# wcy199705/DfFintheWild

Measured on AMD Instinct MI355X. Metric: focal-stacks/sec (10x3x256x256), higher is better.
Workload: dtype bf16x3 (split-bf16 MFMA operands hi+lo, fp32 accumulate, fp32-accurate); 1 GPU; DFF_net forward, 10-slice 3x256x256 focal stacks, batch 32 per GPU (BASELINE.json config 3), dense focus_dists, synthetic weights seed 0; batch_per_gpu=32, global_batch=32, slices=10, height=256, width=256, parallelism=single GPU, precision=bf16x3, input=float32 (B,3,N,H,W), the reference's tensor contract

## Files before the change

dffinthewild_amd/csrc/dffw_dispatch.cpp:

```cpp
#include "dffw_run.h"
#include "dffw_stem.h"

namespace dffw {
namespace {

struct ConvLaunch {
    char kernel[96];
    const char *suffix;
    ConvArgs a;
    RollArgs r;
    int v0, v1;
    double flops, bytes;
};

enum { F_TILE = 100, F_GATHER = 101 };

struct ConvPlan {
    int family = -1;
    int n = 0;
    ConvLaunch l[4];
    bool clear_scores = false;
    const TileCfg *cfg = nullptr;
    TileArgs t;
    bool stem_pipe = false;
// ... 441 lines not shown
    }
    const PackedConv &pc = it->second;
    const LayerDef &L = pc.def;
    const int cin = in0.C + (o.in1 ? o.in1->C : 0);
    if (cin != pc.cin_all) {
        err = fail(DFFW_EINVAL, "layer %s expects %d input channels, got %d", name.c_str(), pc.cin_all, cin);
        return out;
    }
    int Ho, Wo;
    if (L.transposed) {
        Ho = in0.H * 2;
        Wo = in0.W * 2;
    } else {
        const int win = (L.kh == 9 && L.cin == 3) ? in0.W - 2 : in0.W;
        Ho = (in0.H + 2 * L.ph - L.dh * (L.kh - 1) - 1) / L.sh + 1;
        Wo = (win + 2 * L.pw - L.dw * (L.kw - 1) - 1) / L.sw + 1;
    }
    const int No = in0.N + 2 * L.pd - (L.kd - 1);
    if (o.outf == nullptr && !o.discard && !o.sums) out = act(in0.B, No, Ho, Wo, L.cout);
    else { out.B = in0.B; out.N = No; out.H = Ho; out.W = Wo; out.C = L.cout; }
    if (o.out_pre) *o.out_pre = act(in0.B, No, Ho, Wo, L.cout);
    if (!ok()) return out;

    const PackedConv *cls = nullptr;
    if (o.cls) {
        auto ic = e->convs.find(o.cls);
        if (ic != e->convs.end()) cls = &ic->second;
    }
    ConvPlan p;
    plan_conv(name, pc, cls, in0, o, out, sw, e->prec, p);
    if (p.err != DFFW_OK) {
        err = fail(p.err, "%s", p.msg);
        return out;
    }
    float *partial = p.partial_bytes ? (float *)raw(p.partial_bytes) : nullptr;
    if (!ok()) return out;
    if (dry) {
        drop_raw(partial);
        return out;
    }

    const uint16_t *zero = zero_page();
    if (!zero) return out;
    if (p.clear_scores) check(hipMemsetAsync(o.cls_out, 0, (size_t)out.pixels() * 4, s), "score memset");
    const StreamFamily *f = p.family < kStreamCount ? &kStream[p.family] : nullptr;
    const size_t trace_words = p.family == F_TILE ? (size_t)p.t.total_tiles * 8 : (f && f->step_trace) ? STEP_TRACE_WORDS : 0;
    p.t.partial = partial;
    for (int i = 0; i < p.n; ++i) {
        ConvLaunch &l = p.l[i];
        l.a.zero = zero;
        launch(l.kernel, name, l.suffix, l.flops, l.bytes, name.c_str(), trace_words, [&](unsigned long long *trace) {
            l.a.trace = trace;
            if (f) return f->go(e->prec, l, s);
            if (p.family == F_GATHER) return launch_conv(e->prec, l.a, s);
            return p.stem_pipe ? launch_stem_pipe(l.a, p.t, sw.roll_wgs, s) : launch_conv_tile(e->prec, p.cfg, l.a, p.t, s);
        });
    }
    if (partial) {
        launch_unnamed("dffw::splitk_finish_kernel", name, " (split-K finish)", 0.0, p.finish_bytes, "splitk_finish", 0, [&](unsigned long long *) {
#if defined(DFFW_ABL_BUILD) && defined(DFFW_EXP_SKIP_FINISH)
            return hipSuccess;
#endif
            return launch_splitk_finish(e->prec, partial, p.t.ksplit, p.t.partial_stride, p.M_out, pc.nt * 16, L.cout, pc.bias, p.l[0].a.res0, o.relu, out.p, s);
        });
        drop_raw(partial);
    }
    trace_end();
    return out;
}

}
```

dffinthewild_amd/csrc/dffw_engine.cpp:

```cpp
#include <algorithm>
#include <cmath>
#include <cstdarg>
#include <cstdio>
#include <cstdlib>
#include <cstring>
#include <map>
#include <memory>
#include <string>
#include <vector>

#include "dffw_run.h"
#include "dffw_srd_roll.h"
#include "dffw_stem.h"

namespace dffw {

static thread_local std::string g_err;
static thread_local std::string g_last_kernel;
static thread_local std::string g_last_op_kernels;
}
int dffw_fail(int code, const char *fmt, ...) {
    char buf[1024];
    va_list ap;
    va_start(ap, fmt);
// ... 201 lines not shown
                SrdArgs a = srd_args(x.p, out.p, c0->second, c2->second, x.B, x.N, x.H, x.W, sty, stx, r.sw.srd_wgs);
                if (!(a.zero = r.zero_page())) return out;
                a.pooled = with_pool ? pooled->p : nullptr;
                a.w3 = a3->second.w32; a.w1 = a1->second.w32;
                a.w3f = a3->second.watt; a.w1f = a1->second.watt;
                char kn[64];
                const bool pipe16 = x.C == 16 && r.sw.srd_pipe;
                if (pipe16) srd_pipe16_kernel_name(r.e->prec, with_pool, kn, sizeof kn);
                else if (x.C == 16) srd_roll16_kernel_name(r.e->prec, with_pool, kn, sizeof kn);
                else srd_roll_kernel_name(r.e->prec, with_pool, kn, sizeof kn);
                const double px = (double)x.pixels();
                r.launch(kn, p, "", 2.0 * px * (2 * 9 + 4) * x.C * x.C, (with_pool ? 2.25 : 2.0) * px * x.C * r.elem_bytes(), "srd_roll", SRD_TRACE_WORDS, [&](unsigned long long *trace) {
#ifdef DFFW_TRACE_BUILD
                    a.trace = trace;
#endif
                    return pipe16 ? launch_srd_pipe16(r.e->prec, a, r.s) : x.C == 16 ? launch_srd_roll16(r.e->prec, a, r.s) : launch_srd_roll(r.e->prec, a, r.s);
                });
                r.trace_end();
            }
            if (drop_x) r.drop(x);
            return out;
        }
    }
    ConvOpt o1; o1.relu = 1;
    Act t = r.conv(p + ".Focus_Measure.conv.0.0", x, o1);
    ConvOpt o2; o2.relu = 1; o2.res0 = &x;
    Act feat = r.conv(p + ".Focus_Measure.conv.2.0", t, o2);
    r.drop(t);
    if (drop_x) r.drop(x);
    Act out;
    auto i3 = r.e->convs.find(p + ".N_ch_attention.0");
    auto i1 = r.e->convs.find(p + ".N_ch_attention.2");
    if (srd_attention_supported(feat.C) && i3 != r.e->convs.end() && i1 != r.e->convs.end() && i3->second.w32 && i1->second.w32 &&
        !r.sw.on(SW_NO_FUSED_ATTENTION)) {
        out = r.act(feat.B, feat.N, feat.H, feat.W, feat.C);
        const bool with_pool = pooled && !r.sw.on(SW_NO_FUSED_POOL);
        if (with_pool) *pooled = r.act(feat.B, feat.N, feat.H / 2, feat.W / 2, feat.C);
        if (r.ok() && !r.dry) {
            char kn[64];
            snprintf(kn, sizeof kn, "dffw::srd_attention_kernel<%d, %d>", r.e->prec, feat.C);
            const double px = (double)feat.pixels();
            r.launch_unnamed(kn, p, ".N_ch_attention", 2.0 * px * 4 * feat.C * feat.C, (with_pool ? 2.25 : 2.0) * px * feat.C * r.elem_bytes(), "srd_attention", 0, [&](unsigned long long *) {
                return launch_srd_attention(r.e->prec, feat.p, out.p, i3->second.w32, i1->second.w32, feat.B, feat.N, feat.H, feat.W, feat.C, with_pool ? pooled->p : nullptr, r.s);
            });
        }
    } else if (feat.C == 32 && i3 != r.e->convs.end() && i1 != r.e->convs.end() && i3->second.watt && i1->second.watt && feat.W % 16 == 0 &&
               !r.sw.on(SW_NO_FUSED_ATTENTION)) {
        out = r.act(feat.B, feat.N, feat.H, feat.W, feat.C);
        if (r.ok() && !r.dry) {
            char kn[64];
            snprintf(kn, sizeof kn, "dffw::srd_attention_mfma<%d>", r.e->prec);
            const double px = (double)feat.pixels();
            r.launch_unnamed(kn, p, ".N_ch_attention", 2.0 * px * 4 * feat.C * feat.C, 2.0 * px * feat.C * r.elem_bytes(), "srd_attention_mfma", 0, [&](unsigned long long *) {
                return launch_srd_attention_mfma(r.e->prec, feat.p, out.p, i3->second.watt, i1->second.watt, feat.B, feat.N, feat.H, feat.W, r.s);
            });
        }
    } else {
        ConvOpt o3; o3.relu = 1;
        Act a = r.conv(p + ".N_ch_attention.0", feat, o3);
        ConvOpt o4; o4.relu = 2; o4.res0 = &feat;
        out = r.conv(p + ".N_ch_attention.2", a, o4);
        r.drop(a);
    }
    r.drop(feat);
    return out;
}

Act efd(Run &r, const std::string &p, const Act &x, Act *pooled) {
    auto ca = r.e->convs.find(p + ".stride_conv.0"), cb = r.e->convs.find(p + ".max_pooling.1.0");
    const int Ho = x.H / 2, Wo = x.W / 2;
    const double opx = (double)x.B * x.N * Ho * Wo;
    auto fused = [&](int C, int ty, int tx) {
        return x.C == C && pooled && pooled->p && ca != r.e->convs.end() && cb != r.e->convs.end() && x.H % 2 == 0 && x.W % 2 == 0 && Ho % ty == 0 && Wo % tx == 0 &&
               (int64_t)x.B * (Ho / ty) * (Wo / tx) >= r.sw.roll_min_units && !r.sw.on(SW_NO_ROLL) && !r.sw.on(SW_NO_FUSED_EFD) && !r.sw.on(SW_NO_TILE);
    };
    auto args = [&](int cout, uint16_t *out) {
        ConvArgs a;
        memset(&a, 0, sizeof a);
        a.in0 = x.p; a.C0 = x.C;
        a.in1 = pooled->p; a.C1 = x.C;
        a.B = x.B; a.Ni = x.N; a.Hi = x.H; a.Wi = x.W;
        a.Ng = x.N; a.Hg = Ho; a.Wg = Wo;
        a.No = x.N; a.Ho = Ho; a.Wo = Wo;
        a.Cout = cout;
        a.bias = ca->second.bias;
        a.out = out;
        a.relu = 1;
        a.M = (int64_t)x.B * x.N * Ho * Wo;
        return a;
    };
    int ty, tx;
    efd_roll_tile(&ty, &tx);
    if (fused(8, ty, tx) && ca->second.wroll8 && cb->second.wroll8) {
        Act out = r.act(x.B, x.N, Ho, Wo, 16);
        if (r.ok() && !r.dry) {
            ConvArgs a = args(16, out.p);
            if (!(a.zero = r.zero_page())) return out;
            a.dbg = (r.sw.debug_flags & 6) | r.sw.path_bits();
            RollArgs t = roll_args(ca->second.wroll8, x.B, Ho / ty, Wo / tx, 1, r.sw.roll_wgs);
            t.wroll2 = cb->second.wroll8;
            t.bias2 = cb->second.bias;
            char kn[64];
            conv_roll_efd_kernel_name(r.e->prec, a, true, kn, sizeof kn);
            r.launch(kn, p, "", 2.0 * opx * 27.0 * 8 * 16 * 2, ((double)x.pixels() * 8 + opx * 8 + opx * 16) * r.elem_bytes(), "conv_roll_efd", 0,
                     [&](unsigned long long *) { return launch_conv_roll_efd(r.e->prec, a, t, r.s); });
        }
        r.drop(*pooled);
// ... 520 lines not shown
```

dffinthewild_amd/csrc/dffw_internal.h:

```cpp
#pragma once
#include <hip/hip_runtime.h>
#include <stdint.h>

int dffw_fail(int code, const char *fmt, ...);
void dffw_set_last_op_kernels(const char *names);

namespace dffw {

struct Act {
    uint16_t *p = nullptr;
    int B = 0, N = 0, H = 0, W = 0, C = 0;
    int64_t pixels() const { return (int64_t)B * N * H * W; }
};

enum Prec { P_BF16X3 = 0, P_FP16 = 1, P_BF16 = 2 };
inline int prec_parts(int prec) { return prec == P_BF16X3 ? 2 : 1; }

struct TapEntry {
    int dz, dy, dx;
    int coff;
};
static_assert(sizeof(TapEntry) == 16, "TapEntry must be 16 bytes");

#define DFFW_TAP_INVALID (1 << 20)

struct RawStack {
    const void *p;
    int dtype;
    int64_t sb, sn, sy, sx, sc;
    int h, w;
};

#define DFFW_RAW_NORM_F64_BIT 16
#define DFFW_ARGS_RAW 8
#define DFFW_ARGS_SUMS 128
#define DFFW_ARGS_NO_SMALL 32
#define DFFW_ARGS_NO_LEAN_TILE 16
#define DFFW_ARGS_NO_LEAN_ROLL 64
#define DFFW_ARGS_NO_ROLLX 256
#define DFFW_ARGS_NO_SLICE32 1024
#define DFFW_ARGS_NO_ROLLT 2048
#define DFFW_ARGS_NO_ROLLK 512
struct ConvArgs {
    const uint16_t *in0, *in1;
    int C0, C1;
    int B, Ni, Hi, Wi;
    int Ng, Hg, Wg;
    int sy, sx;
    int No, Ho, Wo;
    int osy, osx, ooy, oox;
    int Cout, KC;
    const TapEntry *tab;
    const uint16_t *wpk;
    const float *bias;
    const uint16_t *res0, *res1;
    int res_bcast;
    uint16_t *out;
    uint16_t *out_pre;
    float *outf;
    int outf_ch;
    int64_t outf_plane;
    const float *cls_w;
    float *cls_out;
    int relu;
    int dbg;
    const uint16_t *zero;
    const float *fs32;
    unsigned long long *trace;
    int64_t M;
};

int conv_nt_for(int cout);
hipError_t launch_conv(int prec, const ConvArgs &a, hipStream_t s);
void conv_kernel_name_for(int prec, const ConvArgs &a, char *buf, int n);
hipError_t launch_set_raw(const RawStack &rs, RawStack *dst, hipStream_t s);
hipError_t launch_stack_in(int prec, const float *FS, uint16_t *out, int B, int N, int H, int W, hipStream_t s);
hipError_t launch_from_ncdhw(int prec, const float *x, uint16_t *out, int B, int C, int N, int H, int W, hipStream_t s);
hipError_t launch_to_ncdhw(int prec, const uint16_t *x, float *out, int B, int C, int N, int H, int W, hipStream_t s);
hipError_t launch_pool(int prec, int mode, int k, const uint16_t *x, uint16_t *out, int B, int N, int H, int W, int C, hipStream_t s);
hipError_t launch_pool3(int prec, const uint16_t *x, uint16_t *o2, uint16_t *o4, uint16_t *o8, int B, int N, int H, int W, int C, hipStream_t s);
bool srd_attention_supported(int C);
hipError_t launch_srd_attention(int prec, const uint16_t *feat, uint16_t *out, const float *w3, const float *w1, int B, int N,
                                int H, int W, int C, uint16_t *pooled, hipStream_t s);
hipError_t launch_splitk_finish(int prec, const float *partial, int ksplit, int64_t stride, int64_t M, int cpad, int Cout,
                                const float *bias, const uint16_t *res0, int relu, uint16_t *out, hipStream_t s);
hipError_t launch_from_ncdhw_pad(int prec, const float *x, uint16_t *out, int B, int Cs, int C, int N, int H, int W, hipStream_t s);
hipError_t launch_flow_volume(int prec, const uint16_t *fe, uint16_t *out, const float *alpha, const float *fov, int B, int N,
                              int H, int W, int C, int mode, hipStream_t s);
hipError_t launch_alpha_mean(const float *head, float *alpha, float *raw, int B, int N, int64_t hw, hipStream_t s);
int head_tail_chunks(int B, int N, int64_t hw);
hipError_t launch_head_tail_rows(const float *rows, double *seg, int tiles_x, const float *w, float *alpha, float *raw, int B, int N, int H, int W,
                                 int C, hipStream_t s);
int64_t head_tail_tiles_scratch_bytes(int B, int N, int C);
hipError_t launch_head_tail_tiles(const float *tsum, double *seg, int tiles_y, int tiles_x, const float *w, float *alpha, float *raw, int B,
                                  int N, int H, int W, int C, hipStream_t s);
hipError_t launch_head_tail(int prec, const uint16_t *v, double *partial, const float *w, float *alpha, float *raw, int B, int N, int H, int W,
                            int C, hipStream_t s);
hipError_t launch_fov_warp(const float *x, const float *alpha, const float *fov, float *out, float *flow, int B, int C, int N,
                           int H, int W, int alpha_from_sample0, hipStream_t s);
struct RegressHeads {
    const float *score[4];
    float *depth[4];
    int h[4], w[4];
    int n;
    int nofuse;
};
int regress_form(const RegressHeads &hd, int B, int N, int H, int W);
const char *regress_kernel_name(const RegressHeads &hd, int B, int N, int H, int W);
hipError_t launch_regress_heads(const RegressHeads &hd, int B, int N, int H, int W, const float *fd, int64_t fsb, int64_t fsn, int64_t fsh,
                                int64_t fsw, hipStream_t s);
hipError_t launch_regress(const float *score, int B, int N, int h, int w, int H, int W, const float *fd,
                          int64_t fsb, int64_t fsn, int64_t fsh, int64_t fsw, float *depth, hipStream_t s);

}
```

dffinthewild_amd/csrc/dffw_kernels.hip:

```cpp
#include <cstdio>
#include <cstdlib>

#include "dffw_device.h"
#include "dffw_internal.h"
#include "dffw_persist.h"

namespace dffw {

template <int PREC, int NT, int MT>
__global__ __launch_bounds__(256) void conv_igemm(const ConvArgs a) {
    constexpr int PARTS = Fmt<PREC>::PARTS;
    constexpr bool F16 = (PREC == P_FP16);
    const int lane = threadIdx.x & 63;
    const int wave = threadIdx.x >> 6;
    const int g = lane >> 4, r = lane & 15;
    const int64_t pos0 = ((int64_t)blockIdx.x * 4 + wave) * (MT * 16);
    if (pos0 >= a.M) return;

    const int ps0 = PARTS * a.C0, ps1 = PARTS * a.C1;
    const int64_t samp0 = (int64_t)a.Ni * a.Hi * a.Wi * ps0;
    const int64_t samp1 = (int64_t)a.Ni * a.Hi * a.Wi * ps1;

    int pn[MT], py[MT], px[MT], pbase[MT];
    bool pv[MT];
    int64_t opix[MT];
    const uint16_t *s0[MT];
    const uint16_t *s1[MT];
#pragma unroll
    for (int mt = 0; mt < MT; ++mt) {
        const int64_t p = pos0 + mt * 16 + r;
        pv[mt] = p < a.M;
        const int64_t pp = pv[mt] ? p : 0;
        const int x = (int)(pp % a.Wg);
        int64_t t = pp / a.Wg;
        const int y = (int)(t % a.Hg);
        t /= a.Hg;
        const int n = (int)(t % a.Ng);
        const int b = (int)(t / a.Ng);
        pn[mt] = n;
        py[mt] = y * a.sy;
        px[mt] = x * a.sx;
        pbase[mt] = (n * a.Hi + py[mt]) * a.Wi + px[mt];
        s0[mt] = a.in0 + b * samp0;
        s1[mt] = a.in1 + b * samp1;
        opix[mt] = (((int64_t)b * a.No + n) * a.Ho + (y * a.osy + a.ooy)) * a.Wo + (x * a.osx + a.oox);
    }

    f32x4 acc[NT][MT];
#pragma unroll
    for (int nt = 0; nt < NT; ++nt)
#pragma unroll
        for (int mt = 0; mt < MT; ++mt) acc[nt][mt] = f32x4{0.f, 0.f, 0.f, 0.f};

    const short8 *wbase = reinterpret_cast<const short8 *>(a.wpk) + lane;
    const short8 zero8 = short8{0, 0, 0, 0, 0, 0, 0, 0};

    for (int kc = 0; kc < a.KC; ++kc) {
        const TapEntry te = a.tab[kc * 4 + g];
        const bool tvalid = te.coff >= 0;
        const bool second = te.coff >= a.C0;
        const int cc = tvalid ? (second ? te.coff - a.C0 : te.coff) : 0;
        const int ps = second ? ps1 : ps0;
        const int csrc = second ? a.C1 : a.C0;
        const int delta = (te.dz * a.Hi + te.dy) * a.Wi + te.dx;

// ... 96 lines not shown
                f32x4 &pa = (i & 1) ? acc2 : acc, &qa = (i & 1) ? acc : acc2;
                if constexpr (PARTS == 2) {
                    pa = mma<F16>(wf[i][1], xh[i], pa);
                    qa = mma<F16>(wf[i][0], xl[i], qa);
                }
                pa = mma<F16>(wf[i][0], xh[i], pa);
            }
        }
    }
#pragma unroll
    for (int i = 0; i < 4; ++i) acc[i] += acc2[i];
    if constexpr (KS > 1) {
        red[wave][lane] = acc;
        __syncthreads();
        if (wave != 0) return;
#pragma unroll
        for (int w = 1; w < KS; ++w) {
            const f32x4 o = red[w][lane];
            acc[0] += o[0]; acc[1] += o[1]; acc[2] += o[2]; acc[3] += o[3];
        }
    }
    float cls = 0.f;
    epilogue_quad<PREC, false>(a, acc, nt, g, opix, pv, cls, uint4{}, uint4{});
}

static bool conv_small_wanted(const ConvArgs &a) {
    const int64_t tiles = (a.M + 15) / 16;
    return !a.cls_w && tiles <= 4096 && a.KC >= 1;
}

int conv_nt_for(int cout) {
    const int nt = (cout + 15) / 16;
    return nt <= 1 ? 1 : nt <= 2 ? 2 : nt <= 4 ? 4 : 8;
}

using ConvRow = KernelRow<ConvArgs>;
#define R(P) DFFW_ROW(64, conv_small, P, 1), DFFW_ROW(128, conv_small, P, 2), DFFW_ROW(256, conv_small, P, 4), DFFW_ROW(512, conv_small, P, 8)
static const ConvRow kSmall[] = {R(0), R(1), R(2)};
#undef R
struct IgemmRow {
    ConvRow row;
    int mt;
};
#define R_(P, NT, MT) {DFFW_ROW(256, conv_igemm, P, NT, MT), MT}
#define R(P) R_(P, 1, 4), R_(P, 2, 4), R_(P, 4, 4), R_(P, 8, 2)
static const IgemmRow kIgemm[] = {R(0), R(1), R(2)};
#undef R
#undef R_

struct ConvChoice {
    const ConvRow *row;
    dim3 grid;
};
static ConvChoice select_conv(int prec, const ConvArgs &a) {
    const int nt = conv_nt_for(a.Cout);
    if (conv_small_wanted(a) && !(a.dbg & DFFW_ARGS_NO_SMALL))
        return {prec_row(kSmall, prec, 4, a.KC >= 8 ? 3 : a.KC >= 4 ? 2 : a.KC >= 2 ? 1 : 0), dim3((unsigned)((a.M + 15) / 16), (unsigned)nt)};
    const IgemmRow *r = a.Cout <= 8 * 16 ? prec_row(kIgemm, prec, 4, nt == 8 ? 3 : nt == 4 ? 2 : nt == 2 ? 1 : 0) : nullptr;
    if (!r) return {nullptr, dim3()};
    const int64_t per_wg = 4 * r->mt * 16;
    return {&r->row, dim3((unsigned)((a.M + per_wg - 1) / per_wg))};
}

hipError_t launch_conv(int prec, const ConvArgs &a, hipStream_t s) {
    const ConvChoice c = select_conv(prec, a);
    if (!c.row) return hipErrorInvalidValue;
    hipLaunchKernelGGL(c.row->fn, c.grid, dim3(c.row->block), 0, s, a);
    return hipGetLastError();
}

void conv_kernel_name_for(int prec, const ConvArgs &a, char *buf, int n) { copy_row_name(select_conv(prec, a).row, buf, n); }

template <int PREC>
__global__ __launch_bounds__(256) void stack_in_kernel(const float *__restrict__ FS, uint16_t *__restrict__ out, int B,
                                                       int N, int H, int W) {
    constexpr int PARTS = Fmt<PREC>::PARTS;
    const int W2 = W + 2;
    const int64_t plane = (int64_t)N * H * W;
    const int64_t total = (int64_t)B * N * H * W2;
    for (int64_t i = (int64_t)blockIdx.x * blockDim.x + threadIdx.x; i < total; i += (int64_t)gridDim.x * blockDim.x) {
        const int q = (int)(i % W2);
        const int64_t row = i / W2;
        const int64_t b = row / ((int64_t)N * H);
        const int64_t nh = row - b * (int64_t)N * H;
        const float *src = FS + b * 3 * plane + nh * W;
        short8 h = short8{0, 0, 0, 0, 0, 0, 0, 0}, l = h;
#pragma unroll
        for (int c = 0; c < 3; ++c) {
            uint16_t hi, lo;
            Fmt<PREC>::split(q >= 2 ? src[c * plane + q - 2] : 0.f, hi, lo);
            h[c] = (short)hi;
            l[c] = (short)lo;
            Fmt<PREC>::split(q < W ? src[c * plane + q] : 0.f, hi, lo);
            h[4 + c] = (short)hi;
            l[4 + c] = (short)lo;
        }
        short8 *dst = reinterpret_cast<short8 *>(out + i * (PARTS * 8));
        dst[0] = h;
        if constexpr (PARTS == 2) dst[1] = l;
    }
}

template <int PREC>
__global__ __launch_bounds__(256) void from_ncdhw_kernel(const float *__restrict__ x, uint16_t *__restrict__ out, int B,
                                                         int C, int64_t plane) {
    constexpr int PARTS = Fmt<PREC>::PARTS;
    const int64_t total = (int64_t)B * plane * C;
    for (int64_t i = (int64_t)blockIdx.x * blockDim.x + threadIdx.x; i < total; i += (int64_t)gridDim.x * blockDim.x) {
        const int c = (int)(i % C);
        const int64_t pix = i / C;
        const int64_t b = pix / plane, q = pix - b * plane;
        Fmt<PREC>::store(out + pix * (PARTS * C), C, c, x[(b * C + c) * plane + q]);
    }
}

template <int PREC>
__global__ __launch_bounds__(256) void from_ncdhw_pad_kernel(const float *__restrict__ x, uint16_t *__restrict__ out, int B,
                                                             int Cs, int C, int64_t plane) {
    constexpr int PARTS = Fmt<PREC>::PARTS;
    if (C == 8) {
        const int64_t npix = (int64_t)B * plane;
        for (int64_t pix = (int64_t)blockIdx.x * blockDim.x + threadIdx.x; pix < npix; pix += (int64_t)gridDim.x * blockDim.x) {
            const int64_t b = pix / plane, q = pix - b * plane;
            short8 h = short8{0, 0, 0, 0, 0, 0, 0, 0}, l = h;
// ... 948 lines not shown
```

dffinthewild_amd/csrc/dffw_srd_roll.h:

```cpp
#pragma once
#include "dffw_internal.h"

namespace dffw {

struct SrdArgs {
    const uint16_t *x;
    uint16_t *out;
    uint16_t *pooled;
    const uint16_t *w0, *w2;
    const float *b0, *b2;
    const float *w3, *w1;
    const uint16_t *w3f, *w1f;
    const uint16_t *zero;
    int B, N, H, W;
    int tiles_y, tiles_x, total_tiles;
    int wgs;
#ifdef DFFW_TRACE_BUILD
    unsigned long long *trace;
#endif
};

constexpr int SRD_CHUNKS = 3;
void srd_roll_tile(int *ty, int *tx);
hipError_t launch_srd_roll(int prec, const SrdArgs &a, hipStream_t s);
void srd_roll_kernel_name(int prec, bool pool, char *buf, int n);
constexpr int SRD16_CHUNKS = 5;
void srd_roll16_tile(int *ty, int *tx);
hipError_t launch_srd_roll16(int prec, const SrdArgs &a, hipStream_t s);
void srd_roll16_kernel_name(int prec, bool pool, char *buf, int n);
hipError_t launch_srd_pipe16(int prec, const SrdArgs &a, hipStream_t s);
void srd_pipe16_kernel_name(int prec, bool pool, char *buf, int n);

hipError_t launch_srd_attention_mfma(int prec, const uint16_t *feat, uint16_t *out, const uint16_t *w3f, const uint16_t *w1f, int B, int N,
                                     int H, int W, hipStream_t s);

}
```

dffinthewild_amd/csrc/dffw_srd_roll.hip:

```cpp
#include <algorithm>
#include <cstdio>
#include <cstdlib>
#include <type_traits>

#include "dffw_device.h"
#include "dffw_persist.h"
#include "dffw_srd_roll.h"

namespace dffw {

using SrdRow = KernelRow<SrdArgs>;

template <int PREC, bool POOL, int ABL = 0>
__global__ __launch_bounds__(256) __attribute__((amdgpu_waves_per_eu(3))) void srd_roll_kernel(const SrdArgs a, const float *__restrict__ w3g, const float *__restrict__ w1g) {
    constexpr int PARTS = Fmt<PREC>::PARTS;
    constexpr bool F16 = (PREC == P_FP16);
    constexpr int C = 8, TY = 8, TX = 16, NWAVES = 4;
    constexpr int XY = TY + 4, XX = TX + 4, XPIX = XY * XX;
    constexpr int TYT = TY + 2, TXT = TX + 2, TPIX = TYT * TXT;
    constexpr int PIXB = C * 2;
    constexpr int NPIECE = (XPIX + 63) / 64;
    constexpr int PLANEB = NPIECE * 1024;
    constexpr int SLOTB = PARTS * PLANEB;
    constexpr int RX = 4;
// ... 1022 lines not shown
                Fmt<PREC>::join2(h23, l23, m[2], m[3]);
                uint32_t ph01, ph23, pl01, pl23;
#pragma unroll
                for (int i = 0; i < 4; ++i) {
                    uint32_t mu = __float_as_uint(m[i]);
                    mu = max(mu, (uint32_t)__builtin_amdgcn_mov_dpp((int)mu, 0xB1, 0xF, 0xF, true));
                    mu = max(mu, (uint32_t)__builtin_amdgcn_mov_dpp((int)mu, 0x128, 0xF, 0xF, true));
                    m[i] = __uint_as_float(mu);
                }
                Fmt<PREC>::split2(m[0], m[1], ph01, pl01);
                Fmt<PREC>::split2(m[2], m[3], ph23, pl23);
                if constexpr (PARTS == 2) {
                    swap16(ph01, pl01);
                    swap16(ph23, pl23);
                }
                if ((r & 9) == 0 && !(ABL & 32)) {
                    const int64_t pp = (((int64_t)UC.b * a.N + zC) * (a.H / 2) + (UC.gy0 / 2 + (wave >> 1))) * (a.W / 2) + UC.gx0 / 2 + 4 * (wave & 1) + ((r & 7) >> 1);
                    if constexpr (PARTS == 2) *reinterpret_cast<uint4 *>(a.pooled + pp * rec + (g & 1) * C + (g >> 1) * 8) = make_uint4(ph01, ph23, pl01, pl23);
                    else *reinterpret_cast<uint2 *>(a.pooled + pp * rec + g * 4) = make_uint2(ph01, ph23);
                }
            }
            if constexpr (PARTS == 2) {
                swap16(h01, l01);
                swap16(h23, l23);
                if ((ABL & 32) == 0 || h01 == 0x12345u) *reinterpret_cast<uint4 *>(a.out + pix * rec + (g & 1) * C + (g >> 1) * 8) = make_uint4(h01, h23, l01, l23);
            } else {
                *reinterpret_cast<uint2 *>(a.out + pix * rec + g * 4) = make_uint2(h01, h23);
            }
        }
        UC = UB;
        zC = zB;
        UB = UA;
        zB = zA;
        if (hasA) {
            xslot = (xslot + 1 == RX) ? 0 : xslot + 1;
            if (++zA == a.N) {
                zA = 0;
                cuA += wgs_per_xcd;
                if (cuA < uend) UA = decode(cuA);
            }
        }
    }
    asm volatile("s_waitcnt vmcnt(0)" ::: "memory");
}

template <int PREC>
__global__ __launch_bounds__(256) void srd_attention_mfma(const uint16_t *__restrict__ feat, uint16_t *__restrict__ out,
                                                          const uint16_t *__restrict__ w3f, const uint16_t *__restrict__ w1f, int B, int N,
                                                          int H, int W) {
    constexpr int PARTS = Fmt<PREC>::PARTS;
    constexpr bool F16 = (PREC == P_FP16);
    constexpr int C = 32, REC = PARTS * C;
    const int lane = threadIdx.x & 63, g = lane >> 4, r = lane & 15;
    const int64_t strip = (int64_t)blockIdx.x * 4 + (threadIdx.x >> 6);
    const int strips_per_row = W / 16;
    const int64_t nstrips = (int64_t)B * H * strips_per_row;
    if (strip >= nstrips) return;
    const int sx = (int)(strip % strips_per_row);
    const int64_t by = strip / strips_per_row;
    const int y = (int)(by % H), b = (int)(by / H);
    const int64_t hw = (int64_t)H * W;
    const int64_t pix0 = ((int64_t)b * N * H + y) * W + sx * 16 + r;

    short8 w3[3][2][PARTS], w1[2][2][2];
#pragma unroll
    for (int k = 0; k < 3; ++k)
#pragma unroll
        for (int nt = 0; nt < 2; ++nt)
#pragma unroll
            for (int pt = 0; pt < PARTS; ++pt) w3[k][nt][pt] = reinterpret_cast<const short8 *>(w3f)[((k * 2 + nt) * PARTS + pt) * 64 + lane];
#pragma unroll
    for (int c = 0; c < 2; ++c)
#pragma unroll
        for (int fr = 0; fr < PARTS; ++fr)
#pragma unroll
            for (int nt = 0; nt < 2; ++nt) w1[c][fr][nt] = reinterpret_cast<const short8 *>(w1f)[((c * PARTS + fr) * 2 + nt) * 64 + lane];

    auto load = [&](int z, short8 (&f)[PARTS]) {
#pragma unroll
        for (int pt = 0; pt < PARTS; ++pt) f[pt] = short8{0, 0, 0, 0, 0, 0, 0, 0};
        if ((unsigned)z < (unsigned)N) {
            const uint16_t *p = feat + (pix0 + (int64_t)z * hw) * REC + g * 8;
#pragma unroll
            for (int pt = 0; pt < PARTS; ++pt) f[pt] = *reinterpret_cast<const short8 *>(p + pt * C);
        }
    };
    auto load_res = [&](int z, uint2 (&rh)[2], uint2 (&rl)[2]) {
#pragma unroll
        for (int nt = 0; nt < 2; ++nt) {
            rh[nt] = make_uint2(0, 0);
            rl[nt] = make_uint2(0, 0);
            if (z < N) {
                const uint16_t *cp = feat + (pix0 + (int64_t)z * hw) * REC + nt * 16 + g * 4;
                rh[nt] = *reinterpret_cast<const uint2 *>(cp);
                if constexpr (PARTS == 2) rl[nt] = *reinterpret_cast<const uint2 *>(cp + C);
            }
        }
    };
    short8 f[4][PARTS];
    uint2 rh[2][2], rl[2][2];
    load(-1, f[0]);
    load(0, f[1]);
    load(1, f[2]);
    load_res(0, rh[0], rl[0]);
    for (int z = 0; z < N; ++z) {
        load(z + 2, f[3]);
        load_res(z + 1, rh[1], rl[1]);
        f32x4 at[2];
#pragma unroll
        for (int nt = 0; nt < 2; ++nt) {
            at[nt] = f32x4{0.f, 0.f, 0.f, 0.f};
#pragma unroll
            for (int k = 0; k < 3; ++k) {
                if constexpr (PARTS == 2) {
                    at[nt] = mma<F16>(w3[k][nt][1], f[k][0], at[nt]);
                    at[nt] = mma<F16>(w3[k][nt][0], f[k][1], at[nt]);
                }
                at[nt] = mma<F16>(w3[k][nt][0], f[k][0], at[nt]);
            }
        }
        short8 b2[2];
#pragma unroll
        for (int c = 0; c < 2; ++c) {
            uint32_t ah01, ah23, al01, al23;
            Fmt<PREC>::split2(relu_bits(at[c][0]), relu_bits(at[c][1]), ah01, al01);
            Fmt<PREC>::split2(relu_bits(at[c][2]), relu_bits(at[c][3]), ah23, al23);
            typedef unsigned u32x4v __attribute__((ext_vector_type(4)));
            const u32x4v bq = {ah01, ah23, al01, al23};
            b2[c] = __builtin_bit_cast(short8, bq);
        }
        const int64_t pix = pix0 + (int64_t)z * hw;
#pragma unroll
        for (int nt = 0; nt < 2; ++nt) {
            f32x4 o = f32x4{0.f, 0.f, 0.f, 0.f};
#pragma unroll
            for (int c = 0; c < 2; ++c) {
                if constexpr (PARTS == 2) o = mma<F16>(w1[c][1][nt], b2[c], o);
                o = mma<F16>(w1[c][0][nt], b2[c], o);
            }
            float c0, c1, c2, c3;
            Fmt<PREC>::join2(rh[0][nt].x, rl[0][nt].x, c0, c1);
            Fmt<PREC>::join2(rh[0][nt].y, rl[0][nt].y, c2, c3);
            uint32_t h01, h23, l01, l23;
            Fmt<PREC>::split2(c0 + relu_bits(o[0]), c1 + relu_bits(o[1]), h01, l01);
            Fmt<PREC>::split2(c2 + relu_bits(o[2]), c3 + relu_bits(o[3]), h23, l23);
            if constexpr (PARTS == 2) {
                swap16(h01, l01);
                swap16(h23, l23);
                *reinterpret_cast<uint4 *>(out + pix * REC + (g & 1) * C + (nt * 2 + (g >> 1)) * 8) = make_uint4(h01, h23, l01, l23);
            } else {
                *reinterpret_cast<uint2 *>(out + pix * REC + nt * 16 + g * 4) = make_uint2(h01, h23);
            }
        }
#pragma unroll
        for (int pt = 0; pt < PARTS; ++pt) {
            f[0][pt] = f[1][pt];
            f[1][pt] = f[2][pt];
            f[2][pt] = f[3][pt];
        }
#pragma unroll
        for (int nt = 0; nt < 2; ++nt) {
            rh[0][nt] = rh[1][nt];
            rl[0][nt] = rl[1][nt];
        }
    }
}

hipError_t launch_srd_attention_mfma(int prec, const uint16_t *feat, uint16_t *out, const uint16_t *w3f, const uint16_t *w1f, int B, int N,
                                     int H, int W, hipStream_t s) {
    if (W % 16) return hipErrorInvalidValue;
    const int64_t nstrips = (int64_t)B * H * (W / 16);
    const dim3 grid((unsigned)((nstrips + 3) / 4)), block(256);
    switch (prec) {
        case P_BF16X3: hipLaunchKernelGGL((srd_attention_mfma<P_BF16X3>), grid, block, 0, s, feat, out, w3f, w1f, B, N, H, W); break;
        case P_FP16: hipLaunchKernelGGL((srd_attention_mfma<P_FP16>), grid, block, 0, s, feat, out, w3f, w1f, B, N, H, W); break;
        case P_BF16: hipLaunchKernelGGL((srd_attention_mfma<P_BF16>), grid, block, 0, s, feat, out, w3f, w1f, B, N, H, W); break;
        default: return hipErrorInvalidValue;
    }
    return hipGetLastError();
}

void srd_roll_tile(int *ty, int *tx) {
    *ty = 8;
    *tx = 16;
}

#define DFFW_SRD_ROWS(kernel, P)                                                                      \
    {"dffw::" #kernel "<" #P ", false>", kernel<P, false>, 256}, {"dffw::" #kernel "<" #P ", true>", kernel<P, true>, 256}

static const KernelRow<SrdArgs, const float *, const float *> kSrdRoll[] = {
    DFFW_SRD_ROWS(srd_roll_kernel, 0), DFFW_SRD_ROWS(srd_roll_kernel, 1), DFFW_SRD_ROWS(srd_roll_kernel, 2),
};
#ifdef DFFW_ABL_BUILD
#define R(A) {A, DFFW_ROW(256, srd_roll_kernel, 0, true, A)}
static const AblRow<KernelRow<SrdArgs, const float *, const float *>> kSrdRollAbl[] = {R(1), R(2), R(4), R(6), R(7), R(8), R(16), R(32), R(40), R(23)};
#undef R
#endif
static const KernelRow<SrdArgs, const float *, const float *> *select_srd_roll(int prec, bool pool) {
#ifdef DFFW_ABL_BUILD
    if (prec == P_BF16X3 && pool)
        if (const auto *row = abl_row(kSrdRollAbl, "DFFW_SRD_ABL")) return row;
#endif
    return prec_row(kSrdRoll, prec, 2, pool);
}
void srd_roll_kernel_name(int prec, bool pool, char *buf, int n) { copy_row_name(select_srd_roll(prec, pool), buf, n); }
hipError_t launch_srd_roll(int prec, const SrdArgs &a, hipStream_t s) {
    return launch_row(select_srd_roll(prec, a.pooled != nullptr), a.total_tiles, a.wgs > 0 ? a.wgs : 768, 1, s, a, a.w3, a.w1);
}

void srd_roll16_tile(int *ty, int *tx) {
    *ty = 4;
    *tx = 16;
}

static const SrdRow kSrdRoll16[] = {
    DFFW_SRD_ROWS(srd_roll16_kernel, 0), DFFW_SRD_ROWS(srd_roll16_kernel, 1), DFFW_SRD_ROWS(srd_roll16_kernel, 2),
};
#ifdef DFFW_ABL_BUILD
#define R(A) {A, DFFW_ROW(256, srd_roll16_kernel, 0, true, A)}
static const AblRow<SrdRow> kSrdRoll16Abl[] = {R(1), R(2), R(4), R(6), R(7), R(8), R(16), R(32), R(40), R(23)};
#undef R
#endif
static const SrdRow *select_srd_roll16(int prec, bool pool) {
#ifdef DFFW_ABL_BUILD
    if (prec == P_BF16X3 && pool)
        if (const SrdRow *row = abl_row(kSrdRoll16Abl, "DFFW_SRD_ABL")) return row;
#endif
    return prec_row(kSrdRoll16, prec, 2, pool);
}
void srd_roll16_kernel_name(int prec, bool pool, char *buf, int n) { copy_row_name(select_srd_roll16(prec, pool), buf, n); }
hipError_t launch_srd_roll16(int prec, const SrdArgs &a, hipStream_t s) {
    return launch_row(select_srd_roll16(prec, a.pooled != nullptr), a.total_tiles, a.wgs > 0 ? a.wgs : 512, 1, s, a);
// ... 15 lines not shown
```

Before: 4109 stacks/s.

## Make pointwise igemm and SRD attention persistent with cross-unit prefetch

Adds a pointwise (1x1, stride-1) fast path inside conv_igemm that walks pixel tiles in a grid-stride loop with register weights loaded once and next-tile inputs prefetched. The grid for that path is capped at a configurable workgroup count (default 512). The SRD attention MFMA kernel also becomes persistent: each wave walks several strips, prefetching the next strip's slices while finishing the current one, and the grid is sized to resident occupancy. The aim is to amortize weight loads and hide memory latency, at the cost of more register pressure and a possible load imbalance across waves.

```diff
diff --git a/dffinthewild_amd/csrc/dffw_dispatch.cpp b/dffinthewild_amd/csrc/dffw_dispatch.cpp
--- a/dffinthewild_amd/csrc/dffw_dispatch.cpp
+++ b/dffinthewild_amd/csrc/dffw_dispatch.cpp
@@ -517,7 +517,7 @@
         launch(l.kernel, name, l.suffix, l.flops, l.bytes, name.c_str(), trace_words, [&](unsigned long long *trace) {
             l.a.trace = trace;
             if (f) return f->go(e->prec, l, s);
-            if (p.family == F_GATHER) return launch_conv(e->prec, l.a, s);
+            if (p.family == F_GATHER) return launch_conv(e->prec, l.a, sw.roll_wgs, s);
             return p.stem_pipe ? launch_stem_pipe(l.a, p.t, sw.roll_wgs, s) : launch_conv_tile(e->prec, p.cfg, l.a, p.t, s);
         });
     }
diff --git a/dffinthewild_amd/csrc/dffw_engine.cpp b/dffinthewild_amd/csrc/dffw_engine.cpp
--- a/dffinthewild_amd/csrc/dffw_engine.cpp
+++ b/dffinthewild_amd/csrc/dffw_engine.cpp
@@ -277,7 +277,7 @@
             snprintf(kn, sizeof kn, "dffw::srd_attention_mfma<%d>", r.e->prec);
             const double px = (double)feat.pixels();
             r.launch_unnamed(kn, p, ".N_ch_attention", 2.0 * px * 4 * feat.C * feat.C, 2.0 * px * feat.C * r.elem_bytes(), "srd_attention_mfma", 0, [&](unsigned long long *) {
-                return launch_srd_attention_mfma(r.e->prec, feat.p, out.p, i3->second.watt, i1->second.watt, feat.B, feat.N, feat.H, feat.W, r.s);
+                return launch_srd_attention_mfma(r.e->prec, feat.p, out.p, i3->second.watt, i1->second.watt, feat.B, feat.N, feat.H, feat.W, r.sw.srd_wgs, r.s);
             });
         }
     } else {
diff --git a/dffinthewild_amd/csrc/dffw_internal.h b/dffinthewild_amd/csrc/dffw_internal.h
--- a/dffinthewild_amd/csrc/dffw_internal.h
+++ b/dffinthewild_amd/csrc/dffw_internal.h
@@ -71,7 +71,7 @@
 };
 
 int conv_nt_for(int cout);
-hipError_t launch_conv(int prec, const ConvArgs &a, hipStream_t s);
+hipError_t launch_conv(int prec, const ConvArgs &a, int wgs, hipStream_t s);
 void conv_kernel_name_for(int prec, const ConvArgs &a, char *buf, int n);
 hipError_t launch_set_raw(const RawStack &rs, RawStack *dst, hipStream_t s);
 hipError_t launch_stack_in(int prec, const float *FS, uint16_t *out, int B, int N, int H, int W, hipStream_t s);
diff --git a/dffinthewild_amd/csrc/dffw_kernels.hip b/dffinthewild_amd/csrc/dffw_kernels.hip
--- a/dffinthewild_amd/csrc/dffw_kernels.hip
+++ b/dffinthewild_amd/csrc/dffw_kernels.hip
@@ -6,11 +6,93 @@
 #include "dffw_persist.h"
 
 namespace dffw {
+
+__host__ __device__ inline bool conv_pointwise(const ConvArgs &a) {
+    return a.C1 == 0 && a.KC * 32 == a.C0 && a.sy == 1 && a.sx == 1 && a.osy == 1 && a.osx == 1 && a.ooy == 0 && a.oox == 0 && a.Ng == a.Ni &&
+           a.Hg == a.Hi && a.Wg == a.Wi && a.No == a.Ni && a.Ho == a.Hi && a.Wo == a.Wi;
+}
+__host__ __device__ constexpr int pointwise_tiles(int kc, int nt, int mt) { return kc < 1 || kc > 2 || kc * nt > 8 ? 0 : mt < 2 ? mt : 2; }
+
+template <int PREC, int NT, int MT, int KCN>
+__device__ __forceinline__ void conv_pointwise_walk(const ConvArgs &a) {
+    constexpr int PARTS = Fmt<PREC>::PARTS;
+    constexpr bool F16 = (PREC == P_FP16);
+    constexpr int FT = pointwise_tiles(KCN, NT, MT);
+    const int lane = threadIdx.x & 63, g = lane >> 4, r = lane & 15;
+    const int rec = PARTS * a.C0;
+    const short8 *wbase = reinterpret_cast<const short8 *>(a.wpk) + lane;
+    short8 wf[KCN][NT][PARTS];
+#pragma unroll
+    for (int kc = 0; kc < KCN; ++kc)
+#pragma unroll
+        for (int nt = 0; nt < NT; ++nt)
+#pragma unroll
+            for (int pt = 0; pt < PARTS; ++pt) wf[kc][nt][pt] = wbase[(kc * NT * PARTS + nt * PARTS + pt) * 64];
+
+    const short8 zero8 = short8{0, 0, 0, 0, 0, 0, 0, 0};
+    auto request = [&](int64_t pos, short8 (&xh)[FT][KCN], short8 (&xl)[FT][KCN]) {
+#pragma unroll
+        for (int mt = 0; mt < FT; ++mt) {
+            const int64_t p = pos + mt * 16 + r;
+            const uint16_t *src = a.in0 + p * rec + g * 8;
+#pragma unroll
+            for (int kc = 0; kc < KCN; ++kc) {
+                xh[mt][kc] = zero8;
+                xl[mt][kc] = zero8;
+                if (p < a.M) {
+                    xh[mt][kc] = *reinterpret_cast<const short8 *>(src + kc * 32);
+                    if constexpr (PARTS == 2) xl[mt][kc] = *reinterpret_cast<const short8 *>(src + kc * 32 + a.C0);
+                }
+            }
+        }
+    };
+    const int64_t step = (int64_t)gridDim.x * 4 * (FT * 16);
+    int64_t pos = ((int64_t)blockIdx.x * 4 + (threadIdx.x >> 6)) * (FT * 16);
+    short8 xh[2][FT][KCN], xl[2][FT][KCN];
+    if (pos < a.M) request(pos, xh[0], xl[0]);
+    for (; pos < a.M; pos += step) {
+        if (pos + step < a.M) request(pos + step, xh[1], xl[1]);
+#pragma unroll
+        for (int mt = 0; mt < FT; ++mt) {
+            f32x4 acc[NT];
+#pragma unroll
+            for (int nt = 0; nt < NT; ++nt) acc[nt] = f32x4{0.f, 0.f, 0.f, 0.f};
+#pragma unroll
+            for (int kc = 0; kc < KCN; ++kc)
+#pragma unroll
+                for (int nt = 0; nt < NT; ++nt) {
+                    if constexpr (PARTS == 2) {
+                        acc[nt] = mma<F16>(wf[kc][nt][1], xh[0][mt][kc], acc[nt]);
+                        acc[nt] = mma<F16>(wf[kc][nt][0], xl[0][mt][kc], acc[nt]);
+                    }
+                    acc[nt] = mma<F16>(wf[kc][nt][0], xh[0][mt][kc], acc[nt]);
+                }
+            const int64_t p = pos + mt * 16 + r;
+            float cls = 0.f;
+#pragma unroll
+            for (int nt = 0; nt < NT; ++nt) epilogue_quad<PREC, false>(a, acc[nt], nt, g, p, p < a.M, cls, uint4{}, uint4{});
+            epilogue_cls(a, cls, g, p, p < a.M);
+        }
+#pragma unroll
+        for (int mt = 0; mt < FT; ++mt)
+#pragma unroll
+            for (int kc = 0; kc < KCN; ++kc) {
+                xh[0][mt][kc] = xh[1][mt][kc];
+                xl[0][mt][kc] = xl[1][mt][kc];
+            }
+    }
+}
 
 template <int PREC, int NT, int MT>
 __global__ __launch_bounds__(256) void conv_igemm(const ConvArgs a) {
     constexpr int PARTS = Fmt<PREC>::PARTS;
     constexpr bool F16 = (PREC == P_FP16);
+    if (conv_pointwise(a)) {
+        if constexpr (pointwise_tiles(1, NT, MT) > 0)
+            if (a.KC == 1) return conv_pointwise_walk<PREC, NT, MT, 1>(a);
+        if constexpr (pointwise_tiles(2, NT, MT) > 0)
+            if (a.KC == 2) return conv_pointwise_walk<PREC, NT, MT, 2>(a);
+    }
     const int lane = threadIdx.x & 63;
     const int wave = threadIdx.x >> 6;
     const int g = lane >> 4, r = lane & 15;
@@ -213,24 +295,26 @@
     const ConvRow *row;
     dim3 grid;
 };
-static ConvChoice select_conv(int prec, const ConvArgs &a) {
+static ConvChoice select_conv(int prec, const ConvArgs &a, int wgs) {
     const int nt = conv_nt_for(a.Cout);
     if (conv_small_wanted(a) && !(a.dbg & DFFW_ARGS_NO_SMALL))
         return {prec_row(kSmall, prec, 4, a.KC >= 8 ? 3 : a.KC >= 4 ? 2 : a.KC >= 2 ? 1 : 0), dim3((unsigned)((a.M + 15) / 16), (unsigned)nt)};
     const IgemmRow *r = a.Cout <= 8 * 16 ? prec_row(kIgemm, prec, 4, nt == 8 ? 3 : nt == 4 ? 2 : nt == 2 ? 1 : 0) : nullptr;
     if (!r) return {nullptr, dim3()};
-    const int64_t per_wg = 4 * r->mt * 16;
-    return {&r->row, dim3((unsigned)((a.M + per_wg - 1) / per_wg))};
-}
-
-hipError_t launch_conv(int prec, const ConvArgs &a, hipStream_t s) {
-    const ConvChoice c = select_conv(prec, a);
+    const int ft = conv_pointwise(a) ? pointwise_tiles(a.KC, nt, r->mt) : 0;
+    const int64_t per_wg = 4 * (ft ? ft : r->mt) * 16;
+    const int64_t grid = (a.M + per_wg - 1) / per_wg;
+    return {&r->row, dim3((unsigned)(ft ? std::min<int64_t>(grid, wgs > 0 ? wgs : 512) : grid))};
+}
+
+hipError_t launch_conv(int prec, const ConvArgs &a, int wgs, hipStream_t s) {
+    const ConvChoice c = select_conv(prec, a, wgs);
     if (!c.row) return hipErrorInvalidValue;
     hipLaunchKernelGGL(c.row->fn, c.grid, dim3(c.row->block), 0, s, a);
     return hipGetLastError();
 }
 
-void conv_kernel_name_for(int prec, const ConvArgs &a, char *buf, int n) { copy_row_name(select_conv(prec, a).row, buf, n); }
+void conv_kernel_name_for(int prec, const ConvArgs &a, char *buf, int n) { copy_row_name(select_conv(prec, a, 0).row, buf, n); }
 
 template <int PREC>
 __global__ __launch_bounds__(256) void stack_in_kernel(const float *__restrict__ FS, uint16_t *__restrict__ out, int B,
diff --git a/dffinthewild_amd/csrc/dffw_srd_roll.h b/dffinthewild_amd/csrc/dffw_srd_roll.h
--- a/dffinthewild_amd/csrc/dffw_srd_roll.h
+++ b/dffinthewild_amd/csrc/dffw_srd_roll.h
@@ -32,6 +32,6 @@
 void srd_pipe16_kernel_name(int prec, bool pool, char *buf, int n);
 
 hipError_t launch_srd_attention_mfma(int prec, const uint16_t *feat, uint16_t *out, const uint16_t *w3f, const uint16_t *w1f, int B, int N,
-                                     int H, int W, hipStream_t s);
+                                     int H, int W, int wgs, hipStream_t s);
 
 }
diff --git a/dffinthewild_amd/csrc/dffw_srd_roll.hip b/dffinthewild_amd/csrc/dffw_srd_roll.hip
--- a/dffinthewild_amd/csrc/dffw_srd_roll.hip
+++ b/dffinthewild_amd/csrc/dffw_srd_roll.hip
@@ -1098,15 +1098,19 @@
     constexpr bool F16 = (PREC == P_FP16);
     constexpr int C = 32, REC = PARTS * C;
     const int lane = threadIdx.x & 63, g = lane >> 4, r = lane & 15;
-    const int64_t strip = (int64_t)blockIdx.x * 4 + (threadIdx.x >> 6);
+    const int wave = __builtin_amdgcn_readfirstlane(threadIdx.x >> 6);
     const int strips_per_row = W / 16;
-    const int64_t nstrips = (int64_t)B * H * strips_per_row;
-    if (strip >= nstrips) return;
-    const int sx = (int)(strip % strips_per_row);
-    const int64_t by = strip / strips_per_row;
-    const int y = (int)(by % H), b = (int)(by / H);
+    const int nstrips = B * H * strips_per_row;
+    const UnitRange ur = persistent_range((nstrips + 3) >> 2);
+    const int send = min(ur.end * 4, nstrips), sstep = ur.step * 4;
+    int strip = ur.first * 4 + wave;
     const int64_t hw = (int64_t)H * W;
-    const int64_t pix0 = ((int64_t)b * N * H + y) * W + sx * 16 + r;
+    auto strip_pixel = [&](int st) {
+        const int sx = st % strips_per_row, by = st / strips_per_row;
+        const int y = by % H, b = by / H;
+        return ((int64_t)b * N * H + y) * W + sx * 16;
+    };
+    const int lane_at = r * REC;
 
     short8 w3[3][2][PARTS], w1[2][2][2];
 #pragma unroll
@@ -1122,22 +1126,23 @@
 #pragma unroll
             for (int nt = 0; nt < 2; ++nt) w1[c][fr][nt] = reinterpret_cast<const short8 *>(w1f)[((c * PARTS + fr) * 2 + nt) * 64 + lane];
 
-    auto load = [&](int z, short8 (&f)[PARTS]) {
-#pragma unroll
-        for (int pt = 0; pt < PARTS; ++pt) f[pt] = short8{0, 0, 0, 0, 0, 0, 0, 0};
-        if ((unsigned)z < (unsigned)N) {
-            const uint16_t *p = feat + (pix0 + (int64_t)z * hw) * REC + g * 8;
+    const short8 zero8 = short8{0, 0, 0, 0, 0, 0, 0, 0};
+    auto load = [&](bool have, int64_t pix, short8 (&f)[PARTS]) {
+#pragma unroll
+        for (int pt = 0; pt < PARTS; ++pt) f[pt] = zero8;
+        if (have) {
+            const uint16_t *p = feat + pix * REC + (lane_at + g * 8);
 #pragma unroll
             for (int pt = 0; pt < PARTS; ++pt) f[pt] = *reinterpret_cast<const short8 *>(p + pt * C);
         }
     };
-    auto load_res = [&](int z, uint2 (&rh)[2], uint2 (&rl)[2]) {
+    auto load_res = [&](bool have, int64_t pix, uint2 (&rh)[2], uint2 (&rl)[2]) {
 #pragma unroll
         for (int nt = 0; nt < 2; ++nt) {
             rh[nt] = make_uint2(0, 0);
             rl[nt] = make_uint2(0, 0);
-            if (z < N) {
-                const uint16_t *cp = feat + (pix0 + (int64_t)z * hw) * REC + nt * 16 + g * 4;
+            if (have) {
+                const uint16_t *cp = feat + pix * REC + (lane_at + nt * 16 + g * 4);
                 rh[nt] = *reinterpret_cast<const uint2 *>(cp);
                 if constexpr (PARTS == 2) rl[nt] = *reinterpret_cast<const uint2 *>(cp + C);
             }
@@ -1145,85 +1150,116 @@
     };
     short8 f[4][PARTS];
     uint2 rh[2][2], rl[2][2];
-    load(-1, f[0]);
-    load(0, f[1]);
-    load(1, f[2]);
-    load_res(0, rh[0], rl[0]);
-    for (int z = 0; z < N; ++z) {
-        load(z + 2, f[3]);
-        load_res(z + 1, rh[1], rl[1]);
-        f32x4 at[2];
-#pragma unroll
-        for (int nt = 0; nt < 2; ++nt) {
-            at[nt] = f32x4{0.f, 0.f, 0.f, 0.f};
-#pragma unroll
-            for (int k = 0; k < 3; ++k) {
+    bool primed = false;
+    int64_t pix0 = strip < send ? strip_pixel(strip) : 0;
+    for (; strip < send; strip += sstep) {
+        const bool next = N >= 2 && strip + sstep < send;
+        const int64_t pixn = next ? strip_pixel(strip + sstep) : pix0;
+        if (!primed) {
+            load(true, pix0, f[1]);
+            load(N > 1, pix0 + hw, f[2]);
+            load_res(true, pix0, rh[0], rl[0]);
+        }
+#pragma unroll
+        for (int pt = 0; pt < PARTS; ++pt) f[0][pt] = zero8;
+        for (int z = 0; z < N; ++z) {
+            const int q = z + 2;
+            load(q < N || next, q < N ? pix0 + (int64_t)q * hw : pixn + (int64_t)(q - N) * hw, f[3]);
+            load_res(z + 1 < N || next, z + 1 < N ? pix0 + (int64_t)(z + 1) * hw : pixn, rh[1], rl[1]);
+            short8 fn[PARTS];
+#pragma unroll
+            for (int pt = 0; pt < PARTS; ++pt) fn[pt] = z + 1 < N ? f[2][pt] : zero8;
+            f32x4 at[2];
+#pragma unroll
+            for (int nt = 0; nt < 2; ++nt) {
+                at[nt] = f32x4{0.f, 0.f, 0.f, 0.f};
+#pragma unroll
+                for (int k = 0; k < 3; ++k) {
+                    const short8(&fk)[PARTS] = k == 2 ? fn : f[k];
+                    if constexpr (PARTS == 2) {
+                        at[nt] = mma<F16>(w3[k][nt][1], fk[0], at[nt]);
+                        at[nt] = mma<F16>(w3[k][nt][0], fk[1], at[nt]);
+                    }
+                    at[nt] = mma<F16>(w3[k][nt][0], fk[0], at[nt]);
+                }
+            }
+            short8 b2[2];
+#pragma unroll
+            for (int c = 0; c < 2; ++c) {
+                uint32_t ah01, ah23, al01, al23;
+                Fmt<PREC>::split2(relu_bits(at[c][0]), relu_bits(at[c][1]), ah01, al01);
+                Fmt<PREC>::split2(relu_bits(at[c][2]), relu_bits(at[c][3]), ah23, al23);
+                typedef unsigned u32x4v __attribute__((ext_vector_type(4)));
+                const u32x4v bq = {ah01, ah23, al01, al23};
+                b2[c] = __builtin_bit_cast(short8, bq);
+            }
+            const int64_t pix = pix0 + (int64_t)z * hw;
+#pragma unroll
+            for (int nt = 0; nt < 2; ++nt) {
+                f32x4 o = f32x4{0.f, 0.f, 0.f, 0.f};
+#pragma unroll
+                for (int c = 0; c < 2; ++c) {
+                    if constexpr (PARTS == 2) o = mma<F16>(w1[c][1][nt], b2[c], o);
+                    o = mma<F16>(w1[c][0][nt], b2[c], o);
+                }
+                float c0, c1, c2, c3;
+                Fmt<PREC>::join2(rh[0][nt].x, rl[0][nt].x, c0, c1);
+                Fmt<PREC>::join2(rh[0][nt].y, rl[0][nt].y, c2, c3);
+                uint32_t h01, h23, l01, l23;
+                Fmt<PREC>::split2(c0 + relu_bits(o[0]), c1 + relu_bits(o[1]), h01, l01);
+                Fmt<PREC>::split2(c2 + relu_bits(o[2]), c3 + relu_bits(o[3]), h23, l23);
                 if constexpr (PARTS == 2) {
-                    at[nt] = mma<F16>(w3[k][nt][1], f[k][0], at[nt]);
-                    at[nt] = mma<F16>(w3[k][nt][0], f[k][1], at[nt]);
-                }
-                at[nt] = mma<F16>(w3[k][nt][0], f[k][0], at[nt]);
-            }
-        }
-        short8 b2[2];
-#pragma unroll
-        for (int c = 0; c < 2; ++c) {
-            uint32_t ah01, ah23, al01, al23;
-            Fmt<PREC>::split2(relu_bits(at[c][0]), relu_bits(at[c][1]), ah01, al01);
-            Fmt<PREC>::split2(relu_bits(at[c][2]), relu_bits(at[c][3]), ah23, al23);
-            typedef unsigned u32x4v __attribute__((ext_vector_type(4)));
-            const u32x4v bq = {ah01, ah23, al01, al23};
-            b2[c] = __builtin_bit_cast(short8, bq);
-        }
-        const int64_t pix = pix0 + (int64_t)z * hw;
-#pragma unroll
-        for (int nt = 0; nt < 2; ++nt) {
-            f32x4 o = f32x4{0.f, 0.f, 0.f, 0.f};
-#pragma unroll
-            for (int c = 0; c < 2; ++c) {
-                if constexpr (PARTS == 2) o = mma<F16>(w1[c][1][nt], b2[c], o);
-                o = mma<F16>(w1[c][0][nt], b2[c], o);
-            }
-            float c0, c1, c2, c3;
-            Fmt<PREC>::join2(rh[0][nt].x, rl[0][nt].x, c0, c1);
-            Fmt<PREC>::join2(rh[0][nt].y, rl[0][nt].y, c2, c3);
-            uint32_t h01, h23, l01, l23;
-            Fmt<PREC>::split2(c0 + relu_bits(o[0]), c1 + relu_bits(o[1]), h01, l01);
-            Fmt<PREC>::split2(c2 + relu_bits(o[2]), c3 + relu_bits(o[3]), h23, l23);
-            if constexpr (PARTS == 2) {
-                swap16(h01, l01);
-                swap16(h23, l23);
-                *reinterpret_cast<uint4 *>(out + pix * REC + (g & 1) * C + (nt * 2 + (g >> 1)) * 8) = make_uint4(h01, h23, l01, l23);
-            } else {
-                *reinterpret_cast<uint2 *>(out + pix * REC + nt * 16 + g * 4) = make_uint2(h01, h23);
-            }
-        }
-#pragma unroll
-        for (int pt = 0; pt < PARTS; ++pt) {
-            f[0][pt] = f[1][pt];
-            f[1][pt] = f[2][pt];
-            f[2][pt] = f[3][pt];
-        }
-#pragma unroll
-        for (int nt = 0; nt < 2; ++nt) {
-            rh[0][nt] = rh[1][nt];
-            rl[0][nt] = rl[1][nt];
-        }
+                    swap16(h01, l01);
+                    swap16(h23, l23);
+                    *reinterpret_cast<uint4 *>(out + pix * REC + (lane_at + (g & 1) * C + (nt * 2 + (g >> 1)) * 8)) = make_uint4(h01, h23, l01, l23);
+                } else {
+                    *reinterpret_cast<uint2 *>(out + pix * REC + (lane_at + nt * 16 + g * 4)) = make_uint2(h01, h23);
+                }
+            }
+#pragma unroll
+            for (int pt = 0; pt < PARTS; ++pt) {
+                f[0][pt] = f[1][pt];
+                f[1][pt] = f[2][pt];
+                f[2][pt] = f[3][pt];
+            }
+#pragma unroll
+            for (int nt = 0; nt < 2; ++nt) {
+                rh[0][nt] = rh[1][nt];
+                rl[0][nt] = rl[1][nt];
+            }
+        }
+        primed = next;
+        pix0 = pixn;
     }
 }
 
+using AttentionRow = KernelRow<const uint16_t *, uint16_t *, const uint16_t *, const uint16_t *, int, int, int, int>;
+static const AttentionRow kAttention[] = {DFFW_ROW(256, srd_attention_mfma, 0), DFFW_ROW(256, srd_attention_mfma, 1), DFFW_ROW(256, srd_attention_mfma, 2)};
+
+static int attention_resident_wgs(int prec) {
+    struct Resident {
+        int wgs[3] = {0, 0, 0};
+        Resident() {
+            int dev = 0, cus = 0;
+            if (hipGetDevice(&dev) != hipSuccess || hipDeviceGetAttribute(&cus, hipDeviceAttributeMultiprocessorCount, dev) != hipSuccess) return;
+            for (int p = 0; p < 3; ++p) {
+                int per_cu = 0;
+                if (hipOccupancyMaxActiveBlocksPerMultiprocessor(&per_cu, kAttention[p].fn, kAttention[p].block, 0) == hipSuccess) wgs[p] = per_cu * cus;
+            }
+        }
+    };
+    static const Resident res;
+    return res.wgs[prec];
+}
+
 hipError_t launch_srd_attention_mfma(int prec, const uint16_t *feat, uint16_t *out, const uint16_t *w3f, const uint16_t *w1f, int B, int N,
-                                     int H, int W, hipStream_t s) {
-    if (W % 16) return hipErrorInvalidValue;
+                                     int H, int W, int wgs, hipStream_t s) {
+    const AttentionRow *row = prec_row(kAttention, prec, 1, 0);
     const int64_t nstrips = (int64_t)B * H * (W / 16);
-    const dim3 grid((unsigned)((nstrips + 3) / 4)), block(256);
-    switch (prec) {
-        case P_BF16X3: hipLaunchKernelGGL((srd_attention_mfma<P_BF16X3>), grid, block, 0, s, feat, out, w3f, w1f, B, N, H, W); break;
-        case P_FP16: hipLaunchKernelGGL((srd_attention_mfma<P_FP16>), grid, block, 0, s, feat, out, w3f, w1f, B, N, H, W); break;
-        case P_BF16: hipLaunchKernelGGL((srd_attention_mfma<P_BF16>), grid, block, 0, s, feat, out, w3f, w1f, B, N, H, W); break;
-        default: return hipErrorInvalidValue;
-    }
-    return hipGetLastError();
+    if (W % 16 || !row || nstrips < 1 || nstrips > (1 << 30)) return hipErrorInvalidValue;
+    const int want = wgs > 0 ? wgs : attention_resident_wgs(prec);
+    if (want < 1) return hipErrorInvalidValue;
+    return launch_row(row, (int)((nstrips + 3) / 4), want, 1, s, feat, out, w3f, w1f, B, N, H, W);
 }
 
 void srd_roll_tile(int *ty, int *tx) {
```

Result: no change. 4100 stacks/s (-0.2%).
